# ria8651/octree-tracer

Measured on AMD Instinct MI355X. Metric: Mrays/sec at 1920x1080, depth-16 SVO; achieved HBM GB/s vs peak, higher is better.
Workload: dtype f32+u32

## Files before the change

include/svo_hip.h:

```cpp
#ifndef SVO_HIP_H
#define SVO_HIP_H

#include <stddef.h>
#include <stdint.h>

#ifdef __cplusplus
extern "C" {
#endif

#define SVO_VOXEL_OFFSET 134217728u

typedef enum svo_status {
    SVO_OK = 0,
    SVO_ERR_ARG = -1,
    SVO_ERR_HIP = -2,
    SVO_ERR_STATE = -3,
    SVO_ERR_NO_DEVICE = -4,
    SVO_ERR_COMM = -5
} svo_status;

#define SVO_F_PAUSE_ADAPTIVE 1u
#define SVO_F_SHOW_STEPS 2u
#define SVO_F_SHOW_HITS 4u
#define SVO_F_SHADOWS 8u
// ... 90 lines not shown
int svo_gather_wait(svo_ctx *ctx);
int svo_gather_frame_all(int n, svo_ctx *const *ctxs, const void *const *send, size_t bytes, void *recv_on_root, int root);

int svo_assemble_tiles_rgba(svo_ctx *ctx, const uint32_t *gathered_rgba, uint32_t world, uint32_t n_pad, uint32_t width,
                            uint32_t height, uint32_t tile_w, uint32_t tile_h, uint32_t *rgba_frame_out);

int svo_trace_rays(svo_ctx *ctx, const float *rays, size_t n_rays, svo_hit *hits_out);

int svo_last_render_ms(svo_ctx *ctx, float *ms);
int svo_timing_collect(svo_ctx *ctx, float *ms_out, size_t cap, size_t *n_out);

int svo_diag_gather(svo_ctx *ctx, uint32_t stride_bytes, uint32_t n_loads);

int svo_diag_strip_classes(svo_ctx *ctx, uint8_t *host_out, size_t n_strips);

int svo_scan_dispatch(svo_ctx *ctx, uint32_t node_length);
int svo_scan_read(svo_ctx *ctx, uint32_t *sub, uint32_t *n_sub, uint32_t *unsub, uint32_t *n_unsub,
                  size_t capacity);

#ifdef __cplusplus
}
#endif
#endif
```

octree-tracer_amd/_lib.py:

```python
import ctypes as C
import os

import torch

_HERE = os.path.dirname(os.path.abspath(__file__))
LIB_PATH = os.environ.get("SVO_HIP_LIB") or os.path.join(_HERE, "libsvo_hip.so")


class Uniforms(C.Structure):
    _fields_ = [
        ("camera", C.c_float * 16),
        ("camera_inverse", C.c_float * 16),
        ("dimensions", C.c_float * 4),
        ("sun_dir", C.c_float * 4),
        ("flags", C.c_uint32),
        ("misc_value", C.c_float),
    ]


class TerrainParams(C.Structure):
    _fields_ = [
        ("seed", C.c_uint32),
        ("max_depth", C.c_uint32),
        ("cam", C.c_float * 3),
        ("lod_c", C.c_float),
        ("min_depth", C.c_uint32),
        ("max_words", C.c_uint64),
    ]


DEVICE_SYMBOLS = [
    "svo_device_count", "svo_buffer_alloc", "svo_buffer_free", "svo_buffer_read", "svo_ctx_create", "svo_ctx_destroy", "svo_ctx_set_stream", "svo_set_option", "svo_last_error", "svo_sync",
    "svo_nodes_alloc", "svo_nodes_bind_device", "svo_nodes_write", "svo_nodes_scatter", "svo_nodes_read", "svo_nodes_device_ptr", "svo_nodes_share", "svo_nodes_invalidate",
    "svo_comm_unique_id", "svo_comm_init_rank", "svo_comm_init_all", "svo_comm_destroy", "svo_gather_frame", "svo_gather_frame_all", "svo_gather_wait",
    "svo_set_uniforms", "svo_render", "svo_render_host", "svo_render_tiles", "svo_render_secondary", "svo_render_tiles_secondary", "svo_assemble_tiles", "svo_assemble_tiles_packed", "svo_assemble_tiles_rgba", "svo_pack_records", "svo_trace_rays",
    "svo_last_render_ms", "svo_timing_collect", "svo_diag_gather", "svo_diag_strip_classes", "svo_scan_dispatch", "svo_scan_read",
]
HOST_SYMBOLS = [
    "svo_cpu_octree_new", "svo_cpu_octree_free", "svo_cpu_octree_len", "svo_cpu_octree_load_file",
    "svo_cpu_octree_load_vox", "svo_cpu_octree_load_rsvo", "svo_cpu_octree_from_voxels",
    "svo_cpu_octree_put_in_voxel", "svo_cpu_octree_put_in_block", "svo_cpu_octree_find_voxel",
    "svo_cpu_octree_get_node_mask", "svo_cpu_octree_to_octree", "svo_cpu_octree_raw",
    "svo_cpu_octree_generate_mips", "svo_vox_parse", "svo_vox_write", "svo_rsvo_write",
    "svo_octree_new", "svo_octree_from_words", "svo_octree_free", "svo_octree_len", "svo_octree_raw_data",
    "svo_octree_get_node", "svo_octree_subdivide", "svo_octree_unsubdivide", "svo_octree_find_voxel",
    "svo_octree_expanded", "svo_octree_pos_offset", "svo_octree_holes", "svo_octree_set_node", "svo_octree_position", "svo_octree_take_dirty", "svo_camera_matrices",
    "svo_world_new", "svo_world_free", "svo_world_last_error", "svo_world_insert", "svo_world_remove",
    "svo_world_chunk", "svo_world_chunk_ids", "svo_world_find_voxel", "svo_world_generate_mip_tree",
    "svo_world_save_chunk", "svo_world_load_chunk", "svo_world_load", "svo_cpu_octree_bin", "svo_cpu_octree_from_bin",
    "svo_adaptive_subdivide", "svo_adaptive_unsubdivide", "svo_world_expand",
    "svo_gen_terrain", "svo_gen_terrain_height", "svo_gen_fractal", "svo_gen_random", "svo_nodes_max_depth", "svo_nodes_relayout",
# ... 48 lines not shown
    sig("svo_set_uniforms", C.c_int, vp, C.POINTER(Uniforms))
    sig("svo_render", C.c_int, vp, u32, u32, u32, u32, u32, u32, vp, vp)
    sig("svo_render_host", C.c_int, vp, u32, u32, u32, u32, u32, u32, vp, vp)
    sig("svo_render_tiles", C.c_int, vp, u32, u32, u32, u32, u32, u32, vp, vp)
    sig("svo_render_secondary", C.c_int, vp, u32, u32, u32, u32, u32, u32, u32, vp, vp)
    sig("svo_render_tiles_secondary", C.c_int, vp, u32, u32, u32, u32, u32, u32, u32, vp, vp)
    sig("svo_assemble_tiles", C.c_int, vp, vp, u32, u32, u32, u32, u32, u32, vp)
    sig("svo_assemble_tiles_packed", C.c_int, vp, vp, u32, u32, u32, u32, u32, u32, vp)
    sig("svo_assemble_tiles_rgba", C.c_int, vp, vp, u32, u32, u32, u32, u32, u32, vp)
    sig("svo_pack_records", C.c_int, vp, vp, sz, vp)
    sig("svo_trace_rays", C.c_int, vp, vp, sz, vp)
    sig("svo_last_render_ms", C.c_int, vp, fp)
    sig("svo_timing_collect", C.c_int, vp, fp, sz, C.POINTER(sz))
    sig("svo_diag_gather", C.c_int, vp, u32, u32)
    sig("svo_diag_strip_classes", C.c_int, vp, vp, sz)
    sig("svo_scan_dispatch", C.c_int, vp, u32)
    sig("svo_scan_read", C.c_int, vp, vp, C.POINTER(u32), vp, C.POINTER(u32), sz)
    sig("svo_cpu_octree_new", vp, C.c_uint8)
    sig("svo_cpu_octree_free", None, vp)
    sig("svo_cpu_octree_len", sz, vp)
    sig("svo_cpu_octree_load_file", vp, cp, u32, cp, sz)
    sig("svo_cpu_octree_load_vox", vp, cp, sz, cp, sz)
    sig("svo_cpu_octree_load_rsvo", vp, cp, sz, u32, cp, sz)
    sig("svo_cpu_octree_from_voxels", vp, u32, vp, sz, vp, cp, sz)
    sig("svo_cpu_octree_put_in_voxel", None, vp, fp, C.POINTER(C.c_uint8), u32)
    sig("svo_cpu_octree_put_in_block", None, vp, fp, u32, u32)
    sig("svo_cpu_octree_find_voxel", None, vp, fp, i64, C.POINTER(u64), C.POINTER(u32), fp)
    sig("svo_cpu_octree_get_node_mask", None, vp, sz, C.POINTER(C.c_uint8))
    sig("svo_cpu_octree_to_octree", None, vp, vp)
    sig("svo_cpu_octree_raw", None, vp, vp, vp)
# ... 50 lines not shown
```

octree-tracer_amd/csrc/svo_abi.cpp:

```cpp
#include <hip/hip_runtime.h>

#include <cmath>
#include <cstdio>
#include <cstring>
#include <new>
#include <string>
#include <vector>

#include "svo_ctx.h"

int svo_fail(svo_ctx *ctx, int code, const char *what) {
    if (ctx) ctx->err = what;
    return code;
}

int svo_fail_hip(svo_ctx *ctx, hipError_t e, const char *what) {
    if (ctx) ctx->err = std::string(what) + ": " + hipGetErrorString(e);
    return SVO_ERR_HIP;
}

namespace {

constexpr size_t kScanCapacity = 1024000;

// ... 176 lines not shown
    }
    svo::LaunchInfo li{};
    li.variant = stack ? SVO_VARIANT_STACK : SVO_VARIANT_RESTART;
    li.grid_blocks = ctx->grid_blocks;
    li.num_cus = ctx->num_cus;
    li.strip_items = ctx->strip_items;
    li.deep_stack = ctx->tree_depth > (uint32_t)svo::stack_max_depth(false);
    li.occupancy = ctx->occupancy;
    if (stack && ctx->defer_items < wd.n_items) {
        HIP_TRY(ctx, hipStreamSynchronize(ctx->stream));
        if (ctx->defer_buf) (void)hipFree(ctx->defer_buf);
        ctx->defer_buf = nullptr;
        ctx->frame_parity = 0;
        ctx->defer_items = 0;
        size_t want = wd.n_items < (1u << 16) ? (1u << 16) : wd.n_items;
        HIP_TRY(ctx, hipMalloc((void **)&ctx->defer_buf, (svo::kCounterWords + 2 * (want + 1)) * sizeof(uint32_t)));
        HIP_TRY(ctx, hipMemsetAsync(ctx->defer_buf, 0, (svo::kCounterWords + 2 * (want + 1)) * sizeof(uint32_t), ctx->stream));
        ctx->defer_items = want;
    }
    li.counters = ctx->defer_buf;
    li.work_counter = ctx->defer_buf;
    if (ctx->defer_buf) {
        uint32_t *lists = ctx->defer_buf + svo::kCounterWords;
        const size_t stride = ctx->defer_items + 1;
        li.defer = lists + (ctx->frame_parity ? stride : 0);
        li.next_defer_count = lists + (ctx->frame_parity ? 0 : stride);
    }
    const size_t slot = ctx->ev_slots ? (ctx->ev_count % ctx->ev_slots) : 0;
    const bool timed = ctx->ev_slots && opt.sched_slot == 0;
    if (timed) HIP_TRY(ctx, hipEventRecord(ctx->ev[2 * slot], ctx->stream));
    HIP_TRY(ctx, svo::launch_trace(a, li, ctx->stream));
    if (timed) {
        HIP_TRY(ctx, hipEventRecord(ctx->ev[2 * slot + 1], ctx->stream));
        ctx->ev_count++;
    }
    if (stack) {
        const bool same_input = (wd.mode != 2 || opt.sched_slot == 1) && sc.built_nodes_version == ctx->store->version &&
                                memcmp(&sc.built_uniforms, &ctx->uniforms, sizeof(svo_uniforms)) == 0 && sc.age < 64;
        const bool moving = sc.have_prev && memcmp(&sc.prev_uniforms, &ctx->uniforms, sizeof(svo_uniforms)) != 0;
        const bool fed_back = a.balance != nullptr && a.order != nullptr && !filtered;
        const bool rebuild = schedule && (!sc.valid || (sc.order_filtered && !filtered) || (!same_input && sc.age + 1 >= ctx->sched_period) ||
                                          (same_input && sc.floored && !moving) || (same_input && fed_back && sc.balance_frames < 16u));
        const bool shares_only = rebuild && sc.valid && same_input && fed_back && sc.balance_frames < 16u && !(sc.order_filtered && !filtered) &&
                                 !(sc.floored && !moving);
        const bool floor_now = rebuild && !filtered && moving && ctx->motion_floor != 0u && wd.mode == 0 && wd.n_rects == 1u;
        HIP_TRY(ctx, svo::launch_post(a, li, rebuild ? sc.cost : nullptr, sc.order, n_strips, svo::order_list_cap(wd, n_strips),
                                      rebuild && !filtered, ctx->stream, floor_now ? sc.cls_now : nullptr, ctx->motion_floor,
                                      (fed_back && (!same_input || sc.balance_frames < 16u)) ? sc.balance_frames + 1u : 0u, shares_only));
        if (fed_back) sc.balance_frames++;
        if (rebuild && !filtered) sc.floored = floor_now;
        sc.prev_uniforms = ctx->uniforms;
        sc.have_prev = true;
        ctx->frame_parity ^= 1;
        if (rebuild) {
            if (!filtered) sc.order_filtered = false;
            sc.key = wd;
            sc.valid = true;
            sc.age = 0;
            sc.built_uniforms = ctx->uniforms;
            sc.built_nodes_version = ctx->store->version;
        } else if (schedule) {
            sc.age++;
        }
// ... 265 lines not shown
}

int svo_ctx_destroy(svo_ctx *ctx) {
    if (!ctx) return SVO_OK;
    (void)hipSetDevice(ctx->device);
    if (ctx->stream) (void)hipStreamSynchronize(ctx->stream);
    svo_comm_release(ctx);
    release_store(ctx);
    if (ctx->top_table) (void)hipFree(ctx->top_table);
    if (ctx->status) (void)hipFree(ctx->status);
    if (ctx->defer_buf) (void)hipFree(ctx->defer_buf);
    for (auto &sc : ctx->sched) {
        if (sc.cost) (void)hipFree(sc.cost);
        if (sc.cls_now) (void)hipFree(sc.cls_now);
        if (sc.order) (void)hipFree(sc.order);
    }
    for (void *p : {ctx->shade_hits, ctx->shade_aux, ctx->shade_rays, ctx->shade_shadow, ctx->shade_skip, ctx->scatter_buf})
        if (p) (void)hipFree(p);
    if (ctx->scan_sub) (void)hipFree(ctx->scan_sub);
    if (ctx->stage) (void)hipFree(ctx->stage);
    for (hipEvent_t e : ctx->ev) (void)hipEventDestroy(e);
    if (ctx->own_stream) (void)hipStreamDestroy(ctx->own_stream);
    delete ctx;
    return SVO_OK;
}

int svo_ctx_set_stream(svo_ctx *ctx, void *hip_stream, int use_own) {
    if (!ctx) return SVO_ERR_ARG;
    int rc = bind(ctx);
    if (rc) return rc;
// ... 391 lines not shown
    int rc = bind(ctx);
    if (rc) return rc;
    HIP_TRY(ctx, svo::launch_diag_gather(ctx->nodes, (uint32_t)ctx->capacity, stride_bytes / 4, n_loads, ctx->status, ctx->stream));
    return SVO_OK;
}

int svo_diag_strip_classes(svo_ctx *ctx, uint8_t *host_out, size_t n_strips) {
    if (!ctx || (!host_out && n_strips)) return SVO_ERR_ARG;
    const svo_ctx::Sched &sc = ctx->sched[0];
    if (!sc.cls_now || !sc.order_filtered) return fail(ctx, SVO_ERR_STATE, "the last pixel frame was traced without a culling pass");
    if (n_strips > sc.cap) return fail(ctx, SVO_ERR_ARG, "more strips than the last frame had");
    int rc = bind(ctx);
    if (rc || n_strips == 0) return rc;
    HIP_TRY(ctx, hipMemcpyAsync(host_out, sc.cls_now, n_strips, hipMemcpyDeviceToHost, ctx->stream));
    HIP_TRY(ctx, hipStreamSynchronize(ctx->stream));
    return SVO_OK;
}

int svo_scan_dispatch(svo_ctx *ctx, uint32_t node_length) {
    if (!ctx) return SVO_ERR_ARG;
    if (!ctx->nodes) return fail(ctx, SVO_ERR_STATE, "svo_nodes_alloc not called");
    int rc = bind(ctx);
    if (rc) return rc;
    if (!ctx->scan_sub) {
        uint32_t *lists = nullptr;
        HIP_TRY(ctx, hipMalloc((void **)&lists, 2 * kScanCapacity * sizeof(uint32_t)));
        ctx->scan_sub = lists;
        ctx->scan_unsub = lists + kScanCapacity;
        ctx->scan_capacity = kScanCapacity;
        HIP_TRY(ctx, hipMemsetAsync(ctx->scan_sub, 0, sizeof(uint32_t), ctx->stream));
// ... 37 lines not shown
```

octree-tracer_amd/csrc/svo_ctx.h:

```cpp
#pragma once
#include <cstdlib>
#include <hip/hip_runtime.h>

#include <cstdint>
#include <string>
#include <vector>

#include "svo_device.h"
#include "svo_hip.h"

struct svo_node_store {
    int device = 0;
    uint32_t *nodes = nullptr;
    size_t capacity = 0;
    bool owned = false;
    int refs = 1;
    uint64_t version = 1;
    hipEvent_t last_write = nullptr;
    hipStream_t last_writer = nullptr;
};

struct svo_ctx {
    int device = 0;
    int num_cus = 256;
// ... 42 lines not shown
        bool order_filtered = false;
        uint32_t age = 0;
        svo::WorkDesc key{};
        svo_uniforms built_uniforms{};
        uint64_t built_nodes_version = 0;
        svo_uniforms prev_uniforms{};
        bool have_prev = false;
        bool floored = false;
    };
    Sched sched[2];
    bool list_balance = getenv("SVO_NO_LIST_BALANCE") == nullptr;
    uint32_t motion_floor = 0x1204;
    bool schedule = true;
    uint32_t sched_period = 2;
    int frame_parity = 0;
    void *shade_hits = nullptr, *shade_aux = nullptr, *shade_rays = nullptr, *shade_shadow = nullptr, *shade_skip = nullptr;
    size_t shade_hits_bytes = 0, shade_aux_bytes = 0, shade_rays_bytes = 0, shade_shadow_bytes = 0, shade_skip_bytes = 0;
    uint32_t *debug_buf = nullptr;
    uint32_t strip_items = 64;
    bool dynamic_strips = true;
    std::vector<hipEvent_t> ev;
    size_t ev_slots = 0, ev_count = 0;
    std::string err;
};


int svo_fail(svo_ctx *ctx, int code, const char *what);
int svo_fail_hip(svo_ctx *ctx, hipError_t e, const char *what);
void svo_comm_release(svo_ctx *ctx);
```

octree-tracer_amd/csrc/svo_device.h:

```cpp
#pragma once
#include <hip/hip_runtime.h>
#include <stdint.h>

#include "svo_hip.h"

namespace svo {

constexpr uint32_t kVoxelOffset = 134217728u;
constexpr uint32_t kMaxDescent = 31;
constexpr int kTopLevels = 3;
constexpr int kTopEntries = 1 << (3 * kTopLevels);
constexpr int kTopAuxEntries = 8 + 64;
constexpr int kPathBits = 23;
#ifndef SVO_COUNTER_STRIDE
#define SVO_COUNTER_STRIDE 16416
#endif
constexpr int kCounterStride = SVO_COUNTER_STRIDE;
constexpr int kCounterWords = 64 * kCounterStride;


struct WorkDesc {
    uint32_t mode;
    uint32_t x0, y0;
    uint32_t w, h;
// ... 15 lines not shown
    WorkDesc work;
    const float *rays;
    svo_hit *hits;
    uint32_t *rgba;
    float *aux_t;
    uint32_t *status;
    uint32_t refill_min;
    uint32_t cam_shortcut;
    uint32_t *count_nodes;
    const uint32_t *order;
    uint32_t order_cap;
    uint32_t *debug;
    const uint8_t *skip;
    uint32_t *balance;
    svo_hit *shadow_hits;
};

struct LaunchInfo {
    int variant;
    int grid_blocks;
    int num_cus;
    int *occupancy;
    bool deep_stack;
    uint32_t strip_items;
    uint32_t *counters;
    uint32_t *work_counter;
    uint32_t *defer;
    uint32_t *next_defer_count;
};

hipError_t launch_build_top_table(const uint32_t *nodes, uint32_t n_words, uint32_t *top_table,
                                  hipStream_t stream);
hipError_t launch_trace(const TraceArgs &args, const LaunchInfo &li, hipStream_t stream);
int stack_max_depth(bool deep);
constexpr uint32_t kMaxScheduledStrips = 1u << 20;
#ifndef SVO_COST_SHIFT
#define SVO_COST_SHIFT 2
#endif
constexpr uint32_t kCostShift = SVO_COST_SHIFT, kCostClasses = 128u >> SVO_COST_SHIFT;
constexpr uint32_t kOrderHistWords = 64 * kCostClasses;
constexpr uint32_t kBalanceHead = 32, kBalanceSlots = 4096, kBalanceWords = kBalanceHead + kBalanceSlots;
inline uint32_t order_list_cap(const WorkDesc &, uint32_t n_strips) { return (n_strips + 3u) / 4u + kCostClasses; }
hipError_t launch_post(const TraceArgs &args, const LaunchInfo &li, uint8_t *cost, uint32_t *sched, uint32_t n_strips,
                       uint32_t cap, bool build_schedule, hipStream_t stream, uint8_t *moved = nullptr, uint32_t motion_floor = 0,
                       uint32_t balance_update = 0, bool reuse_cost = false);

hipError_t launch_schedule_skipping(const uint8_t *skip, uint32_t n_items, const uint8_t *prev, uint8_t *cls, uint32_t *sched,
                                    uint32_t n_strips, uint32_t cap, hipStream_t stream);
hipError_t launch_schedule_culling(const TraceArgs &args, const uint8_t *prev, uint8_t *cls, uint32_t *sched, uint32_t n_strips,
                                   uint32_t cap, hipStream_t stream);
hipError_t launch_secondary_gen(const TraceArgs &args, const float *aux_t, float *rays, uint8_t *skip, svo_hit *out, uint32_t k_first,
                                uint32_t n_secondary, uint32_t n_records, hipStream_t stream);
hipError_t launch_shade(const TraceArgs &args, const svo_hit *shadow_hits, uint32_t *rgba, hipStream_t stream);
hipError_t launch_diag_gather(const uint32_t *buf, uint32_t n_words, uint32_t stride_words, uint32_t n_loads, uint32_t *sink,
                              hipStream_t stream);
hipError_t launch_scan(uint32_t *nodes, uint32_t n_words, uint32_t node_length, uint32_t *sub, uint32_t *unsub,
                       uint32_t capacity, bool clear_counters, hipStream_t stream);
hipError_t launch_assemble_tiles(const void *gathered, bool packed, svo_hit *frame, uint32_t world, uint32_t n_pad, uint32_t width,
                                 uint32_t height, uint32_t tile_w, uint32_t tile_h, hipStream_t stream);
hipError_t launch_assemble_tiles_rgba(const uint32_t *gathered, uint32_t *frame, uint32_t world, uint32_t n_pad, uint32_t width,
// ... 7 lines not shown
```

octree-tracer_amd/csrc/svo_kernels.hip:

```cpp
#include <hip/hip_runtime.h>

#include "svo_device.h"
#include "svo_trace_fn.h"

#ifndef SVO_WALK_STOP
#define SVO_WALK_STOP 1
#endif
#ifndef SVO_TOP_IN_LDS
#define SVO_TOP_IN_LDS 1
#endif
#ifndef SVO_WALK_TRIPS
#define SVO_WALK_TRIPS 1
#endif
#ifndef SVO_WALK_ASM
#define SVO_WALK_ASM 1
#endif
#ifndef SVO_WALK_LUT
#define SVO_WALK_LUT 2
#endif
#ifndef SVO_WALK_LUT_CNT
#define SVO_WALK_LUT_CNT 1
#endif
#ifndef SVO_DBG_LIGHT
#define SVO_DBG_LIGHT 0
// ... 197 lines not shown
    return *(const TraceArgs *)p;
}

template <int BLOCK, int NS, int K, bool CNT>
struct StackLds {
    static constexpr int top = SVO_TOP_IN_LDS != 0 ? (1 << (3 * K)) : 0;
    static constexpr int lut = top;
    static constexpr int pools = lut + 64;
    static constexpr int counting = pools + (BLOCK / 64) * (kPoolWords * 64);
    static constexpr int stacks = counting + (CNT ? (BLOCK / 64) * kCountQueue + kSatTags + (1 << (3 * K)) / 8 : 0);
    static constexpr int total = stacks + NS * BLOCK;
};
#if defined(__HIP_DEVICE_COMPILE__) && !defined(__gfx950__)
#error "svo_kernels.hip is written for gfx950: the walk relies on its handling of LDS accesses beyond the allocation and on v_rcp_f32 + one Newton step being the IEEE reciprocal (tools/rcptest_gpu.hip)"
#endif

template <int BLOCK, int NS, int K, bool GE, bool DBG, bool CNT, bool SHD>
__global__ __launch_bounds__(BLOCK, NS > 12 ? 4 : (CNT ? SVO_WAVES_PER_SIMD_CNT : ((SHD || (DBG && SVO_DBG_LIGHT == 0)) ? 6 : SVO_WAVES_PER_SIMD))) void trace_stack_kernel(TraceArgs a, uint32_t strip_items,
                                                               uint32_t *work_counter, uint32_t *defer) {
    constexpr bool DBGH = DBG && SVO_DBG_LIGHT == 0;
    constexpr int D = kPathBits;
    constexpr int SBASE = K + 2;
    constexpr int SMAX = K + 1 + NS;
    static_assert(SMAX <= D - 1, "stack deeper than the path codes");
    constexpr int TBL = 1 << (3 * K);
    constexpr bool kTopInLds = SVO_TOP_IN_LDS != 0;
    using Lds = StackLds<BLOCK, NS, K, CNT>;
    constexpr int kLutWords = 64;
    constexpr int LOFF = Lds::lut;
    constexpr int TOFF = Lds::pools;
// ... 137 lines not shown
    uint32_t home = (blockIdx.x % kShards) * kSubs + (blockIdx.x / kShards) % kSubs;
    uint32_t pend = 0;
    uint32_t next, strip_end;
    auto entry_of = [=](uint32_t sh, uint32_t k) -> uint32_t {
        if (order) return k < order[sh] ? order[kShards + sh * a.order_cap + k] : 0xFFFFFFFFu;
        const uint32_t cand = (((k >> 4) * kShards + sh) << 4) | (k & 15u);
        return cand < n_strips ? cand : 0xFFFFFFFFu;
    };
    {
        const uint32_t my_rank = (blockIdx.x / kShards) * (uint32_t)(BLOCK / 64) + __builtin_amdgcn_readfirstlane(tid >> 6);
        const uint32_t s0 = __builtin_amdgcn_readfirstlane(entry_of(blockIdx.x % kShards, my_rank));
        if (s0 != 0xFFFFFFFFu) {
            next = s0 * strip_items;
            strip_end = min(next + strip_items, n_items);
        } else {
            pend = 0x00FFFFFFu;
            next = strip_end = 0xFFFFFFFEu;
        }
    }
    uint32_t pool_n = 0, pool_i = 0;
    uint32_t t_begin = 0, t_dry = 0;
    uint32_t n_rounds = 0, dbg_active = 0, dbg_iters = 0, dbg_refills = 0, dbg_gens = 0;
    uint64_t c_mark = 0;
    if (DBG) t_begin = (uint32_t)__builtin_amdgcn_s_memrealtime();

    float stf = ST_IDLE;
    uint32_t out = 0;
    float P0 = 0, P1 = 0, P2 = 0, Dr0 = 1, Dr1 = 1, Dr2 = 1, Y0 = 1, Y1 = 1, Y2 = 1;
    float S0 = 1, S1 = 1, S2 = 1;
    float dist = 0.0f, tcur = 0.0f;
    float stepsf = 0.0f;
// ... 396 lines not shown
                cam_mu0 = (uint32_t)__builtin_amdgcn_readfirstlane((int)mu0);
                cam_mu1 = (uint32_t)__builtin_amdgcn_readfirstlane((int)mu1);
                cam_mu2 = (uint32_t)__builtin_amdgcn_readfirstlane((int)mu2);
            }
            cam_ok = (uint32_t)D - sh_of((uint32_t)__builtin_amdgcn_readfirstlane(sh)) >= (uint32_t)(SBASE + 2);
            stf = ST_IDLE;
        }
    }

    {
        uint32_t *const bal = fresh_args().balance;
        if (bal != nullptr && blockIdx.x == 0u && tid == 0u) {
            bal[9] = (uint32_t)__builtin_amdgcn_s_memrealtime();
        }
    }
    if (DBG) {
        uint32_t *const ev = fresh_args().debug + 16u * 16384u + 16u * wave_id;
        if (lane == 0u) ev[0] = (uint32_t)__builtin_amdgcn_s_memrealtime();
        if (lane == 0u) ev[15] = (((uint32_t)__builtin_amdgcn_s_getreg((4 - 1) << 11 | 0 << 6 | 20)) << 16) | (uint32_t)__builtin_amdgcn_s_getreg((16 - 1) << 11 | 0 << 6 | 4);
    }
    for (;;) {
        if (DBGH) c_mark = __builtin_amdgcn_s_memtime();
        if (DBG) n_rounds += 1;
        if (DBGH) {
            const uint32_t nd = (uint32_t)__popcll(__ballot(sabs(stf) == ST_DESC));
            (void)nd;
            if (!CNT) dbg_desc_rounds += nd ? 1u : 0u;
        }
        if (sabs(stf) == ST_DESC) {
            descend();
// ... 42 lines not shown
                if (DBG && next == 0xFFFFFFFFu && t_dry == 0) t_dry = (uint32_t)__builtin_amdgcn_s_memrealtime() | 1u;
                if (DBG && !CNT) dbg_desc_start += (uint32_t)(__builtin_amdgcn_s_memtime() - c_w0);
            }
            const bool more = (pool_n != 0u) || (next != 0xFFFFFFFFu);
            if (more) {
                if (DBGH) dbg_refills += 1;
                if (pool_n == 0u) {
                    if (DBG) dbg_gens += 1;
                    if (DBG && dbg_gens <= 14u) {
                        uint32_t *const ev = fresh_args().debug + 16u * 16384u + 16u * wave_id + dbg_gens;
                        if (lane == 0u) ev[0] = (uint32_t)__builtin_amdgcn_s_memrealtime();
                    }
                    const uint64_t c_g0 = DBGH ? __builtin_amdgcn_s_memtime() : 0ull;
                    const TraceArgs &a = fresh_args();
                    const uint32_t q = next + lane;
                    bool alive = false;
                    float gp0 = 0, gp1 = 0, gp2 = 0, gd0 = 1, gd1 = 1, gd2 = 1, gdist = 0;
                    uint32_t gout = 0;
                    if (q < strip_end) {
                        ItemFast it = decode_item_fast(a.work, q);
                        if (a.work.mode == 2 && a.skip && a.skip[q]) it.valid = false;
                        if (it.valid) {
                            RayIn r;
                            if (a.work.mode == 2) {
                                const float *p = a.rays + 6ull * it.out;
                                r = RayIn{p[0], p[1], p[2], p[3], p[4], p[5]};
                            } else {
                                r = gen_ray(a.u, it.px, it.py);
                            }
                            float pos[3], dir[3];
                            if (!ray_enter(r, pos, dir, gdist)) {
                                write_hit(a.hits, it.out, 0u, 0.0f, 0u, 0u, 0u, 0u);
                                if (a.aux_t) a.aux_t[it.out] = 0.0f;
                                if (SHD) reinterpret_cast<uint4 *>(a.shadow_hits)[it.out] = make_uint4(0u, 0u, 0u, 0u);
                            } else if (!(clean_component(pos[0], dir[0]) && clean_component(pos[1], dir[1]) &&
                                         clean_component(pos[2], dir[2]) && fabsf(gdist) <= 1.0e30f)) {
                                uint32_t slot = atomicAdd(&defer[0], 1u);
                                defer[1u + slot] = q;
                            } else {
                                alive = true;
                                gp0 = pos[0]; gp1 = pos[1]; gp2 = pos[2];
                                gd0 = dir[0]; gd1 = dir[1]; gd2 = dir[2];
                                uint32_t ncode = normal_code(truncf(gp0 * 1.000001f)) |
                                                 (normal_code(truncf(gp1 * 1.000001f)) << 2) |
                                                 (normal_code(truncf(gp2 * 1.000001f)) << 4);
                                gout = it.out | (ncode << 26);
                            }
                        }
                    }
                    const uint64_t am = __ballot(alive);
                    if (alive) {
                        const uint32_t slot = __builtin_amdgcn_mbcnt_hi((uint32_t)(am >> 32),
                                                                        __builtin_amdgcn_mbcnt_lo((uint32_t)am, 0u));
                        gd0 *= kScale; gd1 *= kScale; gd2 *= kScale;
                        pool[0 * 64 + slot] = __float_as_uint(gp0 * kScale);
                        pool[1 * 64 + slot] = __float_as_uint(gp1 * kScale);
                        pool[2 * 64 + slot] = __float_as_uint(gp2 * kScale);
                        pool[3 * 64 + slot] = __float_as_uint(gd0);
                        pool[4 * 64 + slot] = __float_as_uint(gd1);
                        pool[5 * 64 + slot] = __float_as_uint(gd2);
                        pool[6 * 64 + slot] = __float_as_uint(gdist);
                        pool[7 * 64 + slot] = gout;
                    }
// ... 193 lines not shown
    if (DBGH) {
#pragma unroll
        for (int o = 32; o > 0; o >>= 1) {
            dbg_desc_iters += (uint32_t)__shfl_xor((int)dbg_desc_iters, o);
            dbg_desc_lanes += (uint32_t)__shfl_xor((int)dbg_desc_lanes, o);
        }
    }
    if (DBGH) {
        uint32_t last = sabs(stf) == ST_PENDING ? (uint32_t)stepsf : 0u;
#pragma unroll
        for (int o = 32; o > 0; o >>= 1) last = max(last, (uint32_t)__shfl_xor((int)last, o));
        dbg_iters = last;
    }
    if (sabs(stf) == ST_PENDING) flush_record(false);
    {
        uint32_t *const bal = fresh_args().balance;
        if (bal != nullptr && tid == 0u && blockIdx.x < kBalanceSlots) bal[kBalanceHead + blockIdx.x] = (uint32_t)__builtin_amdgcn_s_memrealtime();
        if (bal != nullptr && tid == 0u && blockIdx.x == 0u) bal[19] = gridDim.x;
    }
    if (DBG && lane == 0) {
        uint64_t t_end = __builtin_amdgcn_s_memrealtime();
        uint32_t *d = a.debug + 16u * wave_id;
        d[8] = c_refill;
        d[9] = c_desc;
        d[10] = c_step;
        d[11] = c_gen;
        d[12] = dbg_desc_iters;
        d[13] = dbg_desc_lanes;
        d[14] = dbg_desc_rounds;
        d[15] = dbg_desc_start;
// ... 140 lines not shown
        const float r = fminf(fmaxf(mean / T[k], 0.8f), 1.25f);
        w[k] = fminf(fmaxf(w[k] * (1.0f + gain * (r - 1.0f)), 0.6f * 8192.0f), 1.6f * 8192.0f);
        sum += w[k];
    }
    uint32_t acc = 0u;
    float run = 0.0f;
    for (int k = 0; k < 8; k++) {
        bal[k] = acc;
        run += w[k];
        acc = k == 7 ? 65536u : (uint32_t)(run / sum * 65536.0f + 0.5f);
    }
    bal[8] = 65536u;
    bal[18] += 1u;
}

__global__ __launch_bounds__(256) void post_kernel(TraceArgs a, uint32_t *claim_counters, const uint32_t *list,
                                                   uint32_t *next_deferred_count, uint8_t *cost, uint32_t n_strips, uint32_t balance_update) {
    const rsrc_t rs = make_rsrc(a.nodes, a.n_words);
    const bool misc_bool = (a.u.flags & SVO_F_MISC_BOOL) != 0;
    if (blockIdx.x == 0) {
        for (uint32_t i = threadIdx.x; i < 64u; i += 256u) claim_counters[i * (uint32_t)kCounterStride] = 0u;
        if (threadIdx.x == 0) *next_deferred_count = 0u;
        if (a.balance != nullptr && balance_update != 0u) balance_step(a.balance, balance_update <= 6u ? 0.6f : 0.25f, min(a.balance[19], kBalanceSlots), balance_update);
    }
    const uint32_t n_def = list[0];
    for (uint32_t i = blockIdx.x * 256u + threadIdx.x; i < n_def; i += gridDim.x * 256u) {
        const uint32_t q = list[1u + i];
        const float t = trace_one_restart(a, rs, misc_bool, false, q);
        if (a.shadow_hits) {
            const Item it = decode_item(a.work, q);
            const uint4 rec = reinterpret_cast<const uint4 *>(a.hits)[it.out];
            bool traced = false;
            if ((rec.z >> 16) & 1u) {
                float pos[3], dir[3], dist, org[3], nrm[3], sun[3];
                if (ray_enter(item_ray(a, it), pos, dir, dist)) {
                    secondary_origin(pos, dir, rec.z & 0xFFu, rec.w, t, org, nrm);
                    sun_direction(a.u, sun);
                    const RayIn r = {org[0], org[1], org[2], -sun[0], -sun[1], -sun[2]};
                    trace_ray_restart(a, rs, misc_bool, false, r, a.shadow_hits, it.out, nullptr);
                    traced = true;
                }
            }
            if (!traced) reinterpret_cast<uint4 *>(a.shadow_hits)[it.out] = make_uint4(0u, 0u, 0u, 0u);
        }
    }
    if (cost) {
        const uint32_t lane = threadIdx.x & 63u;
        const uint32_t wave = (blockIdx.x * 256u + threadIdx.x) >> 6, n_waves = gridDim.x * 4u;
        for (uint32_t s = wave; s < n_strips; s += n_waves) {
            ItemFast it = decode_item_wave(a.work, s * 64u, lane);
            uint32_t steps = 0;
            if (it.valid) {
                steps = reinterpret_cast<const uint4 *>(a.hits)[it.out].z & 0xFFu;
                if (a.shadow_hits) steps += reinterpret_cast<const uint4 *>(a.shadow_hits)[it.out].z & 0xFFu;
            }
#pragma unroll
            for (int o = 32; o > 0; o >>= 1) steps = max(steps, (uint32_t)__shfl_xor((int)steps, o));
            if (lane == 0) {
                uint32_t c = min(steps >> kCostShift, kCostClasses - 1u);
                cost[s] = (uint8_t)c;
// ... 431 lines not shown
    const int by = (int)(s / bpr), bx = (int)(s - (uint32_t)by * bpr), rows = (int)((n_strips + bpr - 1u) / bpr);
    uint32_t c = in[s], near = 0u;
    if (c < floor_class) {
        for (int dy = -radius; dy <= radius; dy++)
            for (int dx = -radius; dx <= radius; dx++) {
                const int y = by + dy, x = bx + dx;
                if (y < 0 || y >= rows || x < 0 || x >= (int)bpr) continue;
                const uint32_t t = (uint32_t)y * bpr + (uint32_t)x;
                if (t < n_strips && in[t] >= (64u >> kCostShift)) near++;
            }
        if (near >= min_count) c = floor_class;
    }
    out[s] = (uint8_t)c;
}

hipError_t launch_post(const TraceArgs &args, const LaunchInfo &li, uint8_t *cost, uint32_t *sched, uint32_t n_strips,
                       uint32_t cap, bool build_schedule, hipStream_t stream, uint8_t *moved, uint32_t motion_floor, uint32_t balance_update,
                       bool reuse_cost) {
    uint8_t *const measure = reuse_cost ? nullptr : cost;
    uint32_t blocks = measure ? (n_strips + 3u) / 4u : 256u;
    if (blocks > 2048u) blocks = 2048u;
    if (blocks < 16u) blocks = 16u;
    hipLaunchKernelGGL(post_kernel, dim3(blocks), dim3(256), 0, stream, args, li.counters, (const uint32_t *)li.defer,
                       li.next_defer_count, measure, n_strips, balance_update);
    if (cost && build_schedule) {
        const uint8_t *cls = cost;
        if (moved && motion_floor) {
            hipLaunchKernelGGL(strip_danger_kernel, dim3((n_strips + 255u) / 256u), dim3(256), 0, stream, (const uint8_t *)cost, moved, n_strips,
                               args.work.bpr, (int)((motion_floor >> 8) & 15u), (motion_floor >> 12) & 255u, ((motion_floor & 15u) << 3) >> kCostShift);
            cls = moved;
        }
        launch_order_pair(args.work, cls, sched, n_strips, cap, stream, args.balance);
    }
    return hipGetLastError();
}

template <bool PACKED>
__global__ __launch_bounds__(256) void assemble_tiles_kernel(const uint32_t *gathered, uint4 *frame, uint32_t world, uint32_t n_pad,
                                                             uint32_t width, uint32_t height, uint32_t tile_w, uint32_t tile_h) {
    const uint32_t tiles_x = width / tile_w, n = width * height;
    for (uint32_t i = blockIdx.x * 256u + threadIdx.x; i < n; i += gridDim.x * 256u) {
        const uint32_t y = i / width, x = i - y * width;
        const uint32_t ty = y / tile_h, tx = x / tile_w;
        const uint32_t t = ty * tiles_x + tx, r = t % world, k = t / world;
        const uint64_t src = ((uint64_t)r * n_pad + k) * (tile_w * tile_h) + (y - ty * tile_h) * tile_w + (x - tx * tile_w);
        if (PACKED) {
            const uint32_t *p = gathered + 3u * src;
            const uint32_t info = p[2];
// ... 91 lines not shown
```

octree-tracer_amd/gpu.py:

```python
import ctypes as C

from ._lib import SvoError, lib

OPT_VARIANT, OPT_TIMING, OPT_GRID_BLOCKS, OPT_REFILL_MIN, OPT_STRIP_ITEMS, OPT_DYNAMIC_STRIPS, OPT_PRIO_STEPS, OPT_DEBUG_BUFFER, OPT_SCHEDULE, OPT_TREE_DEPTH, OPT_BLOCK_SHAPE, OPT_SCAN_CLEARS_COUNTERS, OPT_FUSED_SHADOWS, OPT_PAIR_TABLE, OPT_CULL, OPT_CAMERA_SHORTCUT, OPT_SCHEDULE_MOTION = range(17)
VARIANT_RESTART, VARIANT_STACK = 0, 1


class Gpu:
    def __init__(self, device=0, stream=None):
        h = C.c_void_p()
        rc = lib().svo_ctx_create(device, C.byref(h))
        if rc != 0:
            raise SvoError(f"svo_ctx_create(device={device}) failed with status {rc} (no usable HIP device?)")
        self._h = h
        self.device = device
        import torch
        self.set_stream(stream if stream is not None else torch.cuda.current_stream(device).cuda_stream)

    @classmethod
    def new(cls, device=0):
        return cls(device)

    def check(self, rc):
        if rc != 0:
# ... 10 lines not shown

    def sync(self):
        self.check(lib().svo_sync(self._h))

    def last_render_ms(self):
        ms = C.c_float()
        self.check(lib().svo_last_render_ms(self._h, C.byref(ms)))
        return ms.value

    def strip_classes(self, n_strips):
        import numpy as np
        out = np.zeros(n_strips, dtype=np.uint8)
        self.check(lib().svo_diag_strip_classes(self._h, out.ctypes.data_as(C.c_void_p), n_strips))
        return out

    def timing_collect(self, cap=65536):
        import numpy as np
        buf = np.empty(cap, dtype=np.float32)
        n = C.c_size_t()
        self.check(lib().svo_timing_collect(self._h, buf.ctypes.data_as(C.POINTER(C.c_float)), cap, C.byref(n)))
        return buf[:n.value].copy()

    @staticmethod
    def comm_unique_id():
        buf = (C.c_uint8 * 128)()
        rc = lib().svo_comm_unique_id(buf)
        if rc != 0:
            raise SvoError(f"svo_comm_unique_id failed with status {rc} (librccl missing?)")
        return bytes(buf)

# ... 30 lines not shown
```

Measured before the change: 9869.

## Trace deferred rays inside trace kernel and skip post launch when idle

Deferred (numerically unclean) rays are now appended per wave as linked chunks and traced by the same wave at the end of the stack trace kernel, instead of by a separate post kernel. Counter re-arming moves into block 0 of the trace kernel using double-banked counters selected by frame parity. The post kernel now only runs when cost measurement or a balance update is needed, and schedule building is split into its own launch. This aims to remove a kernel launch and its dependency bubble on most frames. The cost is more code in the hot kernel, which may add register pressure, plus tail work on the waves that own deferred rays.

```diff
diff --git a/include/svo_hip.h b/include/svo_hip.h
--- a/include/svo_hip.h
+++ b/include/svo_hip.h
@@ -128,6 +128,8 @@
 
 int svo_diag_strip_classes(svo_ctx *ctx, uint8_t *host_out, size_t n_strips);
 
+int svo_diag_launch_counts(svo_ctx *ctx, uint64_t *trace, uint64_t *post);
+
 int svo_scan_dispatch(svo_ctx *ctx, uint32_t node_length);
 int svo_scan_read(svo_ctx *ctx, uint32_t *sub, uint32_t *n_sub, uint32_t *unsub, uint32_t *n_unsub,
                   size_t capacity);
diff --git a/octree-tracer_amd/_lib.py b/octree-tracer_amd/_lib.py
--- a/octree-tracer_amd/_lib.py
+++ b/octree-tracer_amd/_lib.py
@@ -34,7 +34,7 @@
     "svo_nodes_alloc", "svo_nodes_bind_device", "svo_nodes_write", "svo_nodes_scatter", "svo_nodes_read", "svo_nodes_device_ptr", "svo_nodes_share", "svo_nodes_invalidate",
     "svo_comm_unique_id", "svo_comm_init_rank", "svo_comm_init_all", "svo_comm_destroy", "svo_gather_frame", "svo_gather_frame_all", "svo_gather_wait",
     "svo_set_uniforms", "svo_render", "svo_render_host", "svo_render_tiles", "svo_render_secondary", "svo_render_tiles_secondary", "svo_assemble_tiles", "svo_assemble_tiles_packed", "svo_assemble_tiles_rgba", "svo_pack_records", "svo_trace_rays",
-    "svo_last_render_ms", "svo_timing_collect", "svo_diag_gather", "svo_diag_strip_classes", "svo_scan_dispatch", "svo_scan_read",
+    "svo_last_render_ms", "svo_timing_collect", "svo_diag_gather", "svo_diag_strip_classes", "svo_diag_launch_counts", "svo_scan_dispatch", "svo_scan_read",
 ]
 HOST_SYMBOLS = [
     "svo_cpu_octree_new", "svo_cpu_octree_free", "svo_cpu_octree_len", "svo_cpu_octree_load_file",
@@ -113,6 +113,7 @@
     sig("svo_timing_collect", C.c_int, vp, fp, sz, C.POINTER(sz))
     sig("svo_diag_gather", C.c_int, vp, u32, u32)
     sig("svo_diag_strip_classes", C.c_int, vp, vp, sz)
+    sig("svo_diag_launch_counts", C.c_int, vp, C.POINTER(C.c_uint64), C.POINTER(C.c_uint64))
     sig("svo_scan_dispatch", C.c_int, vp, u32)
     sig("svo_scan_read", C.c_int, vp, vp, C.POINTER(u32), vp, C.POINTER(u32), sz)
     sig("svo_cpu_octree_new", vp, C.c_uint8)
diff --git a/octree-tracer_amd/csrc/svo_abi.cpp b/octree-tracer_amd/csrc/svo_abi.cpp
--- a/octree-tracer_amd/csrc/svo_abi.cpp
+++ b/octree-tracer_amd/csrc/svo_abi.cpp
@@ -214,27 +214,30 @@
         ctx->frame_parity = 0;
         ctx->defer_items = 0;
         size_t want = wd.n_items < (1u << 16) ? (1u << 16) : wd.n_items;
-        HIP_TRY(ctx, hipMalloc((void **)&ctx->defer_buf, (svo::kCounterWords + 2 * (want + 1)) * sizeof(uint32_t)));
-        HIP_TRY(ctx, hipMemsetAsync(ctx->defer_buf, 0, (svo::kCounterWords + 2 * (want + 1)) * sizeof(uint32_t), ctx->stream));
+        const size_t words = 2 * (size_t)svo::kCounterWords + 2 * svo::defer_list_words(want);
+        HIP_TRY(ctx, hipMalloc((void **)&ctx->defer_buf, words * sizeof(uint32_t)));
+        HIP_TRY(ctx, hipMemsetAsync(ctx->defer_buf, 0, words * sizeof(uint32_t), ctx->stream));
         ctx->defer_items = want;
     }
-    li.counters = ctx->defer_buf;
-    li.work_counter = ctx->defer_buf;
-    if (ctx->defer_buf) {
-        uint32_t *lists = ctx->defer_buf + svo::kCounterWords;
-        const size_t stride = ctx->defer_items + 1;
-        li.defer = lists + (ctx->frame_parity ? stride : 0);
-        li.next_defer_count = lists + (ctx->frame_parity ? 0 : stride);
+    if (stack) {
+        uint32_t *const banks = ctx->defer_buf, *const lists = ctx->defer_buf + 2 * (size_t)svo::kCounterWords;
+        const size_t stride = svo::defer_list_words(ctx->defer_items);
+        const int p = ctx->frame_parity;
+        li.work_counter = banks + (p ? svo::kCounterWords : 0);
+        li.defer = lists + (p ? stride : 0);
+        a.rearm_counters = banks + (p ? 0 : svo::kCounterWords);
+        a.rearm_defer_count = lists + (p ? 0 : stride);
     }
     const size_t slot = ctx->ev_slots ? (ctx->ev_count % ctx->ev_slots) : 0;
     const bool timed = ctx->ev_slots && opt.sched_slot == 0;
     if (timed) HIP_TRY(ctx, hipEventRecord(ctx->ev[2 * slot], ctx->stream));
     HIP_TRY(ctx, svo::launch_trace(a, li, ctx->stream));
+    if (wd.n_items != 0) ctx->trace_launches++;
     if (timed) {
         HIP_TRY(ctx, hipEventRecord(ctx->ev[2 * slot + 1], ctx->stream));
         ctx->ev_count++;
     }
-    if (stack) {
+    if (stack && wd.n_items != 0) {
         const bool same_input = (wd.mode != 2 || opt.sched_slot == 1) && sc.built_nodes_version == ctx->store->version &&
                                 memcmp(&sc.built_uniforms, &ctx->uniforms, sizeof(svo_uniforms)) == 0 && sc.age < 64;
         const bool moving = sc.have_prev && memcmp(&sc.prev_uniforms, &ctx->uniforms, sizeof(svo_uniforms)) != 0;
@@ -244,9 +247,15 @@
         const bool shares_only = rebuild && sc.valid && same_input && fed_back && sc.balance_frames < 16u && !(sc.order_filtered && !filtered) &&
                                  !(sc.floored && !moving);
         const bool floor_now = rebuild && !filtered && moving && ctx->motion_floor != 0u && wd.mode == 0 && wd.n_rects == 1u;
-        HIP_TRY(ctx, svo::launch_post(a, li, rebuild ? sc.cost : nullptr, sc.order, n_strips, svo::order_list_cap(wd, n_strips),
-                                      rebuild && !filtered, ctx->stream, floor_now ? sc.cls_now : nullptr, ctx->motion_floor,
-                                      (fed_back && (!same_input || sc.balance_frames < 16u)) ? sc.balance_frames + 1u : 0u, shares_only));
+        const bool measure = rebuild && !shares_only;
+        const uint32_t balance_update = (fed_back && (!same_input || sc.balance_frames < 16u)) ? sc.balance_frames + 1u : 0u;
+        if (measure || balance_update != 0u) {
+            HIP_TRY(ctx, svo::launch_post(a, measure ? sc.cost : nullptr, n_strips, balance_update, ctx->stream));
+            ctx->post_launches++;
+        }
+        if (rebuild && !filtered)
+            HIP_TRY(ctx, svo::launch_schedule(a, sc.cost, sc.order, n_strips, svo::order_list_cap(wd, n_strips), ctx->stream,
+                                              floor_now ? sc.cls_now : nullptr, ctx->motion_floor));
         if (fed_back) sc.balance_frames++;
         if (rebuild && !filtered) sc.floored = floor_now;
         sc.prev_uniforms = ctx->uniforms;
@@ -542,6 +551,7 @@
         if (sc.cost) (void)hipFree(sc.cost);
         if (sc.cls_now) (void)hipFree(sc.cls_now);
         if (sc.order) (void)hipFree(sc.order);
+        if (sc.balance) (void)hipFree(sc.balance);
     }
     for (void *p : {ctx->shade_hits, ctx->shade_aux, ctx->shade_rays, ctx->shade_shadow, ctx->shade_skip, ctx->scatter_buf})
         if (p) (void)hipFree(p);
@@ -963,6 +973,13 @@
     if (rc || n_strips == 0) return rc;
     HIP_TRY(ctx, hipMemcpyAsync(host_out, sc.cls_now, n_strips, hipMemcpyDeviceToHost, ctx->stream));
     HIP_TRY(ctx, hipStreamSynchronize(ctx->stream));
+    return SVO_OK;
+}
+
+int svo_diag_launch_counts(svo_ctx *ctx, uint64_t *trace, uint64_t *post) {
+    if (!ctx) return SVO_ERR_ARG;
+    if (trace) *trace = ctx->trace_launches;
+    if (post) *post = ctx->post_launches;
     return SVO_OK;
 }
 
diff --git a/octree-tracer_amd/csrc/svo_ctx.h b/octree-tracer_amd/csrc/svo_ctx.h
--- a/octree-tracer_amd/csrc/svo_ctx.h
+++ b/octree-tracer_amd/csrc/svo_ctx.h
@@ -80,6 +80,7 @@
     bool schedule = true;
     uint32_t sched_period = 2;
     int frame_parity = 0;
+    uint64_t trace_launches = 0, post_launches = 0;
     void *shade_hits = nullptr, *shade_aux = nullptr, *shade_rays = nullptr, *shade_shadow = nullptr, *shade_skip = nullptr;
     size_t shade_hits_bytes = 0, shade_aux_bytes = 0, shade_rays_bytes = 0, shade_shadow_bytes = 0, shade_skip_bytes = 0;
     uint32_t *debug_buf = nullptr;
diff --git a/octree-tracer_amd/csrc/svo_device.h b/octree-tracer_amd/csrc/svo_device.h
--- a/octree-tracer_amd/csrc/svo_device.h
+++ b/octree-tracer_amd/csrc/svo_device.h
@@ -53,6 +53,8 @@
     const uint8_t *skip;
     uint32_t *balance;
     svo_hit *shadow_hits;
+    uint32_t *rearm_counters;
+    uint32_t *rearm_defer_count;
 };
 
 struct LaunchInfo {
@@ -62,11 +64,10 @@
     int *occupancy;
     bool deep_stack;
     uint32_t strip_items;
-    uint32_t *counters;
     uint32_t *work_counter;
     uint32_t *defer;
-    uint32_t *next_defer_count;
 };
+inline size_t defer_list_words(size_t n_items) { return 1 + n_items + 2 * ((n_items + 63) / 64); }
 
 hipError_t launch_build_top_table(const uint32_t *nodes, uint32_t n_words, uint32_t *top_table,
                                   hipStream_t stream);
@@ -80,9 +81,9 @@
 constexpr uint32_t kOrderHistWords = 64 * kCostClasses;
 constexpr uint32_t kBalanceHead = 32, kBalanceSlots = 4096, kBalanceWords = kBalanceHead + kBalanceSlots;
 inline uint32_t order_list_cap(const WorkDesc &, uint32_t n_strips) { return (n_strips + 3u) / 4u + kCostClasses; }
-hipError_t launch_post(const TraceArgs &args, const LaunchInfo &li, uint8_t *cost, uint32_t *sched, uint32_t n_strips,
-                       uint32_t cap, bool build_schedule, hipStream_t stream, uint8_t *moved = nullptr, uint32_t motion_floor = 0,
-                       uint32_t balance_update = 0, bool reuse_cost = false);
+hipError_t launch_post(const TraceArgs &args, uint8_t *cost, uint32_t n_strips, uint32_t balance_update, hipStream_t stream);
+hipError_t launch_schedule(const TraceArgs &args, const uint8_t *cost, uint32_t *sched, uint32_t n_strips, uint32_t cap, hipStream_t stream,
+                           uint8_t *moved = nullptr, uint32_t motion_floor = 0);
 
 hipError_t launch_schedule_skipping(const uint8_t *skip, uint32_t n_items, const uint8_t *prev, uint8_t *cls, uint32_t *sched,
                                     uint32_t n_strips, uint32_t cap, hipStream_t stream);
diff --git a/octree-tracer_amd/csrc/svo_kernels.hip b/octree-tracer_amd/csrc/svo_kernels.hip
--- a/octree-tracer_amd/csrc/svo_kernels.hip
+++ b/octree-tracer_amd/csrc/svo_kernels.hip
@@ -235,6 +235,40 @@
 #if defined(__HIP_DEVICE_COMPILE__) && !defined(__gfx950__)
 #error "svo_kernels.hip is written for gfx950: the walk relies on its handling of LDS accesses beyond the allocation and on v_rcp_f32 + one Newton step being the IEEE reciprocal (tools/rcptest_gpu.hip)"
 #endif
+
+__device__ __forceinline__ void trace_deferred(const TraceArgs &a, rsrc_t rs, bool misc_bool, uint32_t q) {
+    const float t = trace_one_restart(a, rs, misc_bool, false, q);
+    if (a.shadow_hits) {
+        const Item it = decode_item(a.work, q);
+        const uint4 rec = reinterpret_cast<const uint4 *>(a.hits)[it.out];
+        bool traced = false;
+        if ((rec.z >> 16) & 1u) {
+            float pos[3], dir[3], dist, org[3], nrm[3], sun[3];
+            if (ray_enter(item_ray(a, it), pos, dir, dist)) {
+                secondary_origin(pos, dir, rec.z & 0xFFu, rec.w, t, org, nrm);
+                sun_direction(a.u, sun);
+                const RayIn r = {org[0], org[1], org[2], -sun[0], -sun[1], -sun[2]};
+                trace_ray_restart(a, rs, misc_bool, false, r, a.shadow_hits, it.out, nullptr);
+                traced = true;
+            }
+        }
+        if (!traced) reinterpret_cast<uint4 *>(a.shadow_hits)[it.out] = make_uint4(0u, 0u, 0u, 0u);
+    }
+}
+
+template <bool GE>
+__device__ __forceinline__ void trace_deferred_chain(const uint32_t *list, uint32_t head, uint32_t lane) {
+    __threadfence();
+    const TraceArgs &a = fresh_args();
+    const rsrc_t rs = make_rsrc(a.nodes, a.n_words);
+    while (head != 0u) {
+        const uint32_t *chunk = list + head;
+        const uint32_t prev = (uint32_t)__builtin_amdgcn_readfirstlane((int)chunk[0]);
+        const uint32_t n = (uint32_t)__builtin_amdgcn_readfirstlane((int)chunk[1]);
+        if (lane < n) trace_deferred(a, rs, GE, chunk[2u + lane]);
+        head = prev;
+    }
+}
 
 template <int BLOCK, int NS, int K, bool GE, bool DBG, bool CNT, bool SHD>
 __global__ __launch_bounds__(BLOCK, NS > 12 ? 4 : (CNT ? SVO_WAVES_PER_SIMD_CNT : ((SHD || (DBG && SVO_DBG_LIGHT == 0)) ? 6 : SVO_WAVES_PER_SIMD))) void trace_stack_kernel(TraceArgs a, uint32_t strip_items,
@@ -402,7 +436,7 @@
             next = s0 * strip_items;
             strip_end = min(next + strip_items, n_items);
         } else {
-            pend = 0x00FFFFFFu;
+            if (lane == 0u) pend = 0x00FFFFFFu;
             next = strip_end = 0xFFFFFFFEu;
         }
     }
@@ -829,6 +863,11 @@
             bal[9] = (uint32_t)__builtin_amdgcn_s_memrealtime();
         }
     }
+    if (blockIdx.x == 0u) {
+        const TraceArgs &fa = fresh_args();
+        if (tid < 64u) fa.rearm_counters[tid * (uint32_t)kCounterStride] = 0u;
+        else if (tid == 64u) *fa.rearm_defer_count = 0u;
+    }
     if (DBG) {
         uint32_t *const ev = fresh_args().debug + 16u * 16384u + 16u * wave_id;
         if (lane == 0u) ev[0] = (uint32_t)__builtin_amdgcn_s_memrealtime();
@@ -901,7 +940,7 @@
                     const uint64_t c_g0 = DBGH ? __builtin_amdgcn_s_memtime() : 0ull;
                     const TraceArgs &a = fresh_args();
                     const uint32_t q = next + lane;
-                    bool alive = false;
+                    bool alive = false, deferred = false;
                     float gp0 = 0, gp1 = 0, gp2 = 0, gd0 = 1, gd1 = 1, gd2 = 1, gdist = 0;
                     uint32_t gout = 0;
                     if (q < strip_end) {
@@ -922,8 +961,7 @@
                                 if (SHD) reinterpret_cast<uint4 *>(a.shadow_hits)[it.out] = make_uint4(0u, 0u, 0u, 0u);
                             } else if (!(clean_component(pos[0], dir[0]) && clean_component(pos[1], dir[1]) &&
                                          clean_component(pos[2], dir[2]) && fabsf(gdist) <= 1.0e30f)) {
-                                uint32_t slot = atomicAdd(&defer[0], 1u);
-                                defer[1u + slot] = q;
+                                deferred = true;
                             } else {
                                 alive = true;
                                 gp0 = pos[0]; gp1 = pos[1]; gp2 = pos[2];
@@ -934,6 +972,20 @@
                                 gout = it.out | (ncode << 26);
                             }
                         }
+                    }
+                    const uint64_t dm = __ballot(deferred);
+                    if (dm != 0ull) {
+                        const uint32_t nd = (uint32_t)__popcll(dm);
+                        uint32_t base = 0u;
+                        if (lane == 0u) base = atomicAdd(&defer[0], nd + 2u);
+                        base = (uint32_t)__builtin_amdgcn_readfirstlane((int)base);
+                        if (lane == 0u) {
+                            defer[1u + base] = (uint32_t)__builtin_amdgcn_readlane((int)pend, 1);
+                            defer[2u + base] = nd;
+                        }
+                        if (deferred)
+                            defer[3u + base + __builtin_amdgcn_mbcnt_hi((uint32_t)(dm >> 32), __builtin_amdgcn_mbcnt_lo((uint32_t)dm, 0u))] = q;
+                        if (lane == 1u) pend = base + 1u;
                     }
                     const uint64_t am = __ballot(alive);
                     if (alive) {
@@ -1157,6 +1209,10 @@
     }
     if (sabs(stf) == ST_PENDING) flush_record(false);
     {
+        const uint32_t dhead = (uint32_t)__builtin_amdgcn_readlane((int)pend, 1);
+        if (dhead != 0u) trace_deferred_chain<GE>(defer, dhead, lane);
+    }
+    {
         uint32_t *const bal = fresh_args().balance;
         if (bal != nullptr && tid == 0u && blockIdx.x < kBalanceSlots) bal[kBalanceHead + blockIdx.x] = (uint32_t)__builtin_amdgcn_s_memrealtime();
         if (bal != nullptr && tid == 0u && blockIdx.x == 0u) bal[19] = gridDim.x;
@@ -1327,36 +1383,9 @@
     bal[18] += 1u;
 }
 
-__global__ __launch_bounds__(256) void post_kernel(TraceArgs a, uint32_t *claim_counters, const uint32_t *list,
-                                                   uint32_t *next_deferred_count, uint8_t *cost, uint32_t n_strips, uint32_t balance_update) {
-    const rsrc_t rs = make_rsrc(a.nodes, a.n_words);
-    const bool misc_bool = (a.u.flags & SVO_F_MISC_BOOL) != 0;
-    if (blockIdx.x == 0) {
-        for (uint32_t i = threadIdx.x; i < 64u; i += 256u) claim_counters[i * (uint32_t)kCounterStride] = 0u;
-        if (threadIdx.x == 0) *next_deferred_count = 0u;
-        if (a.balance != nullptr && balance_update != 0u) balance_step(a.balance, balance_update <= 6u ? 0.6f : 0.25f, min(a.balance[19], kBalanceSlots), balance_update);
-    }
-    const uint32_t n_def = list[0];
-    for (uint32_t i = blockIdx.x * 256u + threadIdx.x; i < n_def; i += gridDim.x * 256u) {
-        const uint32_t q = list[1u + i];
-        const float t = trace_one_restart(a, rs, misc_bool, false, q);
-        if (a.shadow_hits) {
-            const Item it = decode_item(a.work, q);
-            const uint4 rec = reinterpret_cast<const uint4 *>(a.hits)[it.out];
-            bool traced = false;
-            if ((rec.z >> 16) & 1u) {
-                float pos[3], dir[3], dist, org[3], nrm[3], sun[3];
-                if (ray_enter(item_ray(a, it), pos, dir, dist)) {
-                    secondary_origin(pos, dir, rec.z & 0xFFu, rec.w, t, org, nrm);
-                    sun_direction(a.u, sun);
-                    const RayIn r = {org[0], org[1], org[2], -sun[0], -sun[1], -sun[2]};
-                    trace_ray_restart(a, rs, misc_bool, false, r, a.shadow_hits, it.out, nullptr);
-                    traced = true;
-                }
-            }
-            if (!traced) reinterpret_cast<uint4 *>(a.shadow_hits)[it.out] = make_uint4(0u, 0u, 0u, 0u);
-        }
-    }
+__global__ __launch_bounds__(256) void post_kernel(TraceArgs a, uint8_t *cost, uint32_t n_strips, uint32_t balance_update) {
+    if (blockIdx.x == 0 && a.balance != nullptr && balance_update != 0u)
+        balance_step(a.balance, balance_update <= 6u ? 0.6f : 0.25f, min(a.balance[19], kBalanceSlots), balance_update);
     if (cost) {
         const uint32_t lane = threadIdx.x & 63u;
         const uint32_t wave = (blockIdx.x * 256u + threadIdx.x) >> 6, n_waves = gridDim.x * 4u;
@@ -1818,24 +1847,22 @@
     out[s] = (uint8_t)c;
 }
 
-hipError_t launch_post(const TraceArgs &args, const LaunchInfo &li, uint8_t *cost, uint32_t *sched, uint32_t n_strips,
-                       uint32_t cap, bool build_schedule, hipStream_t stream, uint8_t *moved, uint32_t motion_floor, uint32_t balance_update,
-                       bool reuse_cost) {
-    uint8_t *const measure = reuse_cost ? nullptr : cost;
-    uint32_t blocks = measure ? (n_strips + 3u) / 4u : 256u;
+hipError_t launch_post(const TraceArgs &args, uint8_t *cost, uint32_t n_strips, uint32_t balance_update, hipStream_t stream) {
+    uint32_t blocks = cost ? (n_strips + 3u) / 4u : 1u;
     if (blocks > 2048u) blocks = 2048u;
-    if (blocks < 16u) blocks = 16u;
-    hipLaunchKernelGGL(post_kernel, dim3(blocks), dim3(256), 0, stream, args, li.counters, (const uint32_t *)li.defer,
-                       li.next_defer_count, measure, n_strips, balance_update);
-    if (cost && build_schedule) {
-        const uint8_t *cls = cost;
-        if (moved && motion_floor) {
-            hipLaunchKernelGGL(strip_danger_kernel, dim3((n_strips + 255u) / 256u), dim3(256), 0, stream, (const uint8_t *)cost, moved, n_strips,
-                               args.work.bpr, (int)((motion_floor >> 8) & 15u), (motion_floor >> 12) & 255u, ((motion_floor & 15u) << 3) >> kCostShift);
-            cls = moved;
-        }
-        launch_order_pair(args.work, cls, sched, n_strips, cap, stream, args.balance);
-    }
+    hipLaunchKernelGGL(post_kernel, dim3(blocks), dim3(256), 0, stream, args, cost, n_strips, balance_update);
+    return hipGetLastError();
+}
+
+hipError_t launch_schedule(const TraceArgs &args, const uint8_t *cost, uint32_t *sched, uint32_t n_strips, uint32_t cap, hipStream_t stream,
+                           uint8_t *moved, uint32_t motion_floor) {
+    const uint8_t *cls = cost;
+    if (moved && motion_floor) {
+        hipLaunchKernelGGL(strip_danger_kernel, dim3((n_strips + 255u) / 256u), dim3(256), 0, stream, cost, moved, n_strips,
+                           args.work.bpr, (int)((motion_floor >> 8) & 15u), (motion_floor >> 12) & 255u, ((motion_floor & 15u) << 3) >> kCostShift);
+        cls = moved;
+    }
+    launch_order_pair(args.work, cls, sched, n_strips, cap, stream, args.balance);
     return hipGetLastError();
 }
 
diff --git a/octree-tracer_amd/gpu.py b/octree-tracer_amd/gpu.py
--- a/octree-tracer_amd/gpu.py
+++ b/octree-tracer_amd/gpu.py
@@ -48,6 +48,11 @@
         self.check(lib().svo_diag_strip_classes(self._h, out.ctypes.data_as(C.c_void_p), n_strips))
         return out
 
+    def launch_counts(self):
+        trace, post = C.c_uint64(), C.c_uint64()
+        self.check(lib().svo_diag_launch_counts(self._h, C.byref(trace), C.byref(post)))
+        return trace.value, post.value
+
     def timing_collect(self, cap=65536):
         import numpy as np
         buf = np.empty(cap, dtype=np.float32)
```

Result: faster. 10000, median of 6 (+1.3%).
